# myungsub/meta-interpolation

Measured on AMD Instinct MI355X. Metric: inner-loop steps/sec, higher is better.
Workload: dtype f32 (3x3 convolutions: Winograd F(4x4) / F(2x2) on exact-f32 MFMAs, csrc/winograd4.h + winograd.hip; weight gradients and 5x5 / 7x7 / direct layers on csrc/convk*.hip: bf16x6 split operands, f32 accumulate; 51-tap op on 8-bit frames: exact integer frames x bf16x3 split taps, f32 accumulate); 1 GPU; c2_sepconv_256x448_b4_s5; plugin=sepconv, tasks_per_gpu=4, global_meta_batch=4, inner_steps=5, frame=256x448x3, inner_rule=lslr+SGD, seeded_weights=default, parallelism=task-parallel x1, 1 all-reduce of outer grads

## Files before the change

### meta-interpolation_amd/csrc/convk_wgrad.hip

```cpp
#include "common.h"
#include <stdlib.h>
#include <algorithm>

typedef float f32x4 __attribute__((ext_vector_type(4)));
typedef short bf16x8 __attribute__((ext_vector_type(8)));
typedef short bf16x4 __attribute__((ext_vector_type(4)));
typedef unsigned u32x4 __attribute__((ext_vector_type(4)));
typedef int i32x4 __attribute__((ext_vector_type(4)));
__device__ float ckw_raw_buffer_load_f32(i32x4 rsrc, int voffset, int soffset, int aux) __asm("llvm.amdgcn.raw.buffer.load.f32");

namespace {

constexpr int WG_THREADS = 256;
constexpr int UR = 4, UW = 32;

__device__ __forceinline__ i32x4 ckw_rsrc(const void* base, unsigned bytes) {
  const unsigned long long p = reinterpret_cast<unsigned long long>(base);
  i32x4 r;
  r.x = (int)(unsigned)p;
  r.y = (int)(unsigned)(p >> 32);
  r.z = (int)bytes;
  r.w = 0x00020000;
  return r;
}
// ... 570 lines not shown
  else wgrad_reduce_block(partial, gw, n, splits, blockIdx.x);
}

struct WgPlan { int mt, nt, ng, cobs, cibs, units, upr, ups, splits, ups_per_split, form; };

inline int savfi_cu_count() {
  static int cus[32] = {0};
  int dev = 0;
  if (hipGetDevice(&dev) != hipSuccess) return 256;
  int& n = cus[dev & 31];
  if (n == 0) {
    int v = 0;
    n = (hipDeviceGetAttribute(&v, hipDeviceAttributeMultiprocessorCount, dev) == hipSuccess && v > 0) ? v : 256;
  }
  return n;
}

inline int wg_plan(WgPlan& p, int N, int T, int Ci, int Co, int H, int W, int K, int pad, bool precise) {
  if (N <= 0 || T <= 0 || Ci <= 0 || Co <= 0 || H <= 0 || W <= 0 || N % T != 0 || pad < 0 || pad > K - 1) return SAVFI_E_SHAPE;
  if (K != 3 && K != 5 && K != 7) return SAVFI_E_UNSUPPORTED;
  const int Ho = H + 2 * pad - K + 1, Wo = W + 2 * pad - K + 1;
  if (Ho <= 0 || Wo <= 0) return SAVFI_E_SHAPE;
  if ((int64_t)Ci * H * W >= (1ll << 29) || (int64_t)Co * Ho * Wo >= (1ll << 29)) return SAVFI_E_TOOBIG;
  p.mt = (K == 3 && Co >= 192) ? 4 : 2;
#ifdef SAVFI_WGRAD_MT4
  if (K == 3 && Co >= SAVFI_WGRAD_MT4) p.mt = 4;
#endif
  p.nt = 1;
#if defined(SAVFI_WGRAD_NT) && SAVFI_WGRAD_NT == 2
  if (!precise && K != 7 && p.mt == 2 && Ci > 16) p.nt = 2;
#endif
  p.ng = 1;
#if defined(SAVFI_WGRAD_NG) && SAVFI_WGRAD_NG == 2
  if (K == 3 && p.mt == 4 && !precise && Ci >= 32) p.ng = 2;
#endif
#ifndef SAVFI_WGRAD3_FORM
#define SAVFI_WGRAD3_FORM 2
#endif
  p.form = (K == 3 && !precise && Co >= 48 && Ci >= 48 && SAVFI_WGRAD3_FORM == 2) ? 2 : 0;
  if (p.form) { p.mt = 4; p.nt = 4; p.ng = 1; }
  p.cobs = (Co + 16 * p.mt - 1) / (16 * p.mt);
  p.cibs = (Ci + 16 * p.nt * p.ng - 1) / (16 * p.nt * p.ng);
  const int ur = p.form == 2 ? ring::UR2 : UR;
  p.upr = (Ho + ur - 1) / ur;
  p.ups = (Wo + UW - 1) / UW;
  p.units = (N / T) * p.upr * p.ups;
  const int blocks = T * p.cobs * p.cibs;
  int splits;
#ifndef SAVFI_WGRAD_TARGET
#define SAVFI_WGRAD_TARGET 0
#endif
  constexpr int target = SAVFI_WGRAD_TARGET;
  if (target > 0) {
    splits = (target + blocks - 1) / blocks;
  } else {
    const int per_cu = (p.ng == 2 || p.form) ? 1 : (K == 3 && p.mt == 2 && p.nt == 1 && !precise) ? 3 : 2;
    const int64_t slots = (int64_t)per_cu * savfi_cu_count();
    double best_cost = 0.0;
    splits = 1;
    const int smax = (int)std::min<int64_t>(p.units, 4 * slots / blocks + 1);
    for (int sp = 1; sp <= smax; ++sp) {
      const int ups = (p.units + sp - 1) / sp;
      if ((p.units + ups - 1) / ups != sp) continue;
      const int64_t rounds = ((int64_t)blocks * sp + slots - 1) / slots;
      const double cost = p.form == 2 ? (double)rounds * (ups + 3.0) + 0.12 * sp : (double)rounds * (ups + 1.0) + 0.06 * sp;
      if (sp == 1 || cost < best_cost) { best_cost = cost; splits = sp; }
    }
  }
  if (splits > p.units) splits = p.units;
  if (splits < 1) splits = 1;
  p.ups_per_split = (p.units + splits - 1) / splits;
  p.splits = (p.units + p.ups_per_split - 1) / p.ups_per_split;
  return SAVFI_OK;
}

int launch_wgrad3_ring(const WgArgs& a, int blocks, float* bias_partial, hipStream_t stream) {
  static uint32_t configured = 0, configured_b = 0;
  const int rc = bias_partial ? savfi_ensure_dynamic_lds(reinterpret_cast<const void*>(convk_wgrad3_ring<true>), ring::LDS, configured_b)
                              : savfi_ensure_dynamic_lds(reinterpret_cast<const void*>(convk_wgrad3_ring<false>), ring::LDS, configured);
  if (rc != SAVFI_OK) return rc;
  if (bias_partial) hipLaunchKernelGGL(convk_wgrad3_ring<true>, dim3(blocks), dim3(ring::NTHR), ring::LDS, stream, a, bias_partial);
  else hipLaunchKernelGGL(convk_wgrad3_ring<false>, dim3(blocks), dim3(ring::NTHR), ring::LDS, stream, a, bias_partial);
  return savfi_launch_status();
}

template <int KS, int MT, int NT, bool P2 = false, int NG = 1>
int launch_wgrad(const WgArgs& a, int blocks, hipStream_t stream) {
  using G = WgGeom<KS, MT, NT * NG>;
  static uint32_t configured = 0;
  auto kern = convk_wgrad_kernel<KS, MT, NT, P2, NG>;
  if (G::LDS > 64 * 1024) {
    const int rc = savfi_ensure_dynamic_lds(reinterpret_cast<const void*>(kern), G::LDS, configured);
    if (rc != SAVFI_OK) return rc;
  }
  hipLaunchKernelGGL(kern, dim3(blocks), dim3(WG_THREADS * NG), G::LDS, stream, a);
  return savfi_launch_status();
}

}

extern "C" int64_t savfi_convk_wgrad_workspace_floats(int N, int T, int Ci, int Co, int H, int W, int K, int pad) {
  WgPlan p, q;
  int rc = wg_plan(p, N, T, Ci, Co, H, W, K, pad, false);
  if (rc != SAVFI_OK) return rc;
  rc = wg_plan(q, N, T, Ci, Co, H, W, K, pad, true);
  if (rc != SAVFI_OK) return rc;
  return (int64_t)(p.splits > q.splits ? p.splits : q.splits) * T * Co * (Ci * K * K + 1);
}

extern "C" int savfi_convk_wgrad_sums_bias(int N, int T, int Ci, int Co, int H, int W, int K, int pad) {
  WgPlan p;
  return wg_plan(p, N, T, Ci, Co, H, W, K, pad, false) == SAVFI_OK && p.form == 2 ? 1 : 0;
}

extern "C" int savfi_convk_wgrad_tasks_f32(const float* x, const float* gz, float* gw, float* workspace, int N, int T, int Ci, int Co,
                                           int H, int W, int K, int pad, int precise, void* stream) {
  return savfi_convk_wgrad_tasks_reflect_f32(x, gz, gw, workspace, N, T, Ci, Co, H, W, K, pad, precise, 0, stream);
}

namespace {
int convk_wgrad_run(const float* x, const float* gz, float* gw, float* gb, float* workspace, int N, int T, int Ci, int Co, int H, int W, int K,
                    int pad, int precise, int reflect, void* stream);
}

extern "C" int savfi_convk_wgrad_tasks_reflect_f32(const float* x, const float* gz, float* gw, float* workspace, int N, int T, int Ci,
                                                   int Co, int H, int W, int K, int pad, int precise, int reflect, void* stream) {
  return convk_wgrad_run(x, gz, gw, nullptr, workspace, N, T, Ci, Co, H, W, K, pad, precise, reflect, stream);
}

extern "C" int savfi_convk_wgrad_tasks_bias_f32(const float* x, const float* gz, float* gw, float* gb, float* workspace, int N, int T, int Ci,
                                                int Co, int H, int W, int K, int pad, int reflect, void* stream) {
  if (!gb) return SAVFI_E_NULL;
  if (!savfi_convk_wgrad_sums_bias(N, T, Ci, Co, H, W, K, pad)) return SAVFI_E_UNSUPPORTED;
  return convk_wgrad_run(x, gz, gw, gb, workspace, N, T, Ci, Co, H, W, K, pad, 0, reflect, stream);
}

namespace {
int convk_wgrad_run(const float* x, const float* gz, float* gw, float* gb, float* workspace, int N, int T, int Ci, int Co, int H, int W, int K,
                    int pad, int precise, int reflect, void* stream) {
  if (reflect && (pad >= H || pad >= W)) return SAVFI_E_UNSUPPORTED;
  if (!x || !gz || !gw || !workspace) return SAVFI_E_NULL;
  WgPlan p;
  int rc = wg_plan(p, N, T, Ci, Co, H, W, K, pad, precise != 0);
  if (rc != SAVFI_OK) return rc;
  WgArgs a;
  a.x = x; a.gz = gz; a.partial = workspace;
  a.N = N; a.T = T; a.Ci = Ci; a.Co = Co; a.H = H; a.W = W; a.pad = pad; a.reflect = reflect ? 1 : 0;
  a.Ho = H + 2 * pad - K + 1; a.Wo = W + 2 * pad - K + 1;
  a.cobs = p.cobs; a.cibs = p.cibs; a.splits = p.splits; a.units = p.units; a.units_per_split = p.ups_per_split;
  a.upr = p.upr; a.ups = p.ups;
  const int blocks = T * p.cobs * p.cibs * p.splits;
  hipStream_t st = (hipStream_t)stream;
  float* bias_partial = gb ? workspace + (size_t)p.splits * T * Co * Ci * K * K : nullptr;
  if (p.form == 2) rc = launch_wgrad3_ring(a, blocks, bias_partial, st);
  else if (K == 3 && precise) rc = p.mt == 4 ? launch_wgrad<3, 4, 1, true>(a, blocks, st) : launch_wgrad<3, 2, 1, true>(a, blocks, st);
  else if (K == 3 && p.ng == 2) rc = launch_wgrad<3, 4, 1, false, 2>(a, blocks, st);
  else if (K == 3) rc = p.mt == 4 ? launch_wgrad<3, 4, 1>(a, blocks, st) : p.nt == 2 ? launch_wgrad<3, 2, 2>(a, blocks, st) : launch_wgrad<3, 2, 1>(a, blocks, st);
  else if (K == 5) rc = precise ? launch_wgrad<5, 2, 1, true>(a, blocks, st) : p.nt == 2 ? launch_wgrad<5, 2, 2>(a, blocks, st) : launch_wgrad<5, 2, 1>(a, blocks, st);
  else rc = launch_wgrad<7, 2, 1>(a, blocks, st);
  if (rc != SAVFI_OK) return rc;
  const long long n = (long long)T * Co * Ci * K * K;
  const bool v4 = n % 4 == 0 && (((uintptr_t)workspace | (uintptr_t)gw) & 15u) == 0;
  const long long nb = gb ? (long long)T * Co : 0;
  const unsigned main_blocks = (unsigned)(v4 ? (n / 4 + 31) / 32 : (n + 31) / 32), bias_blocks = (unsigned)((nb + 31) / 32);
  if (v4) hipLaunchKernelGGL(convk_wgrad_reduce<true>, dim3(main_blocks + bias_blocks), dim3(256), 0, st, workspace, gw, n, p.splits, main_blocks, bias_partial, gb, nb);
  else hipLaunchKernelGGL(convk_wgrad_reduce<false>, dim3(main_blocks + bias_blocks), dim3(256), 0, st, workspace, gw, n, p.splits, main_blocks, bias_partial, gb, nb);
  return savfi_launch_status();
}
}
```

### meta-interpolation_amd/csrc/wgrad.hip

```cpp
#include "common.h"

namespace {

typedef float f32x4 __attribute__((ext_vector_type(4)));

constexpr int GNT = 256;
constexpr int GCO = 32, GCI = 32, GSEG = 64;
constexpr int GP = 68;
constexpr int G_FLOATS = GCO * GP;
constexpr int X_FLOATS = 3 * GCI * GP;
constexpr int BUF_FLOATS = G_FLOATS + X_FLOATS;
constexpr int TILE_FLOATS = 2 * 2 * 9 * 256;
constexpr int LDS_FLOATS_G = (2 * BUF_FLOATS > TILE_FLOATS) ? 2 * BUF_FLOATS : TILE_FLOATS;

struct WgradArgs {
  const float* x;
  const float* gz;
  float* partial;
  int Ci, Co, H, W, Ho, Wo, pad, rows, nseg, nrowchunk, cibs;
  int T;
};

struct Staged {
  float g[8], x[3][8], halo;
// ... 116 lines not shown
          acc[1][0][t] = __builtin_amdgcn_mfma_f32_16x16x4f32(ga1[ks], xs[0][ks + b], acc[1][0][t], 0, 0, 0);
          acc[1][1][t] = __builtin_amdgcn_mfma_f32_16x16x4f32(ga1[ks], xs[1][ks + b], acc[1][1][t], 0, 0, 0);
        }
    }
    store_rows(nxt, st, cols, tid, w);
    __syncthreads();
  }

  float* red = lds + lane * 4;
  for (int turn = 0; turn < 4; ++turn) {
    if (w == turn) {
#pragma unroll
      for (int rb = 0; rb < 2; ++rb)
#pragma unroll
        for (int cb = 0; cb < 2; ++cb)
#pragma unroll
          for (int t = 0; t < 9; ++t) {
            float* p = red + ((rb * 2 + cb) * 9 + t) * 256;
            f32x4 v = acc[rb][cb][t];
            if (turn > 0) v += *reinterpret_cast<const f32x4*>(p);
            if (turn < 3) *reinterpret_cast<f32x4*>(p) = v;
            else acc[rb][cb][t] = v;
          }
    }
    __syncthreads();
  }
  if (w == 3) {
    float* out = a.partial + (((size_t)blockIdx.z * gridDim.x + blockIdx.x) * gridDim.y + blockIdx.y) * TILE_FLOATS + lane * 4;
#pragma unroll
    for (int rb = 0; rb < 2; ++rb)
#pragma unroll
      for (int cb = 0; cb < 2; ++cb)
#pragma unroll
        for (int t = 0; t < 9; ++t) *reinterpret_cast<f32x4*>(out + ((rb * 2 + cb) * 9 + t) * 256) = acc[rb][cb][t];
  }
}

constexpr int RG = 16;
__global__ __launch_bounds__(256) void wgrad_reduce1(const float* __restrict__ partial, float* __restrict__ stage2,
                                                     size_t block_floats, int nsplit) {
  const size_t e4 = (size_t)blockIdx.x * 256 + threadIdx.x;
  if (e4 * 4 >= block_floats) return;
  partial += (size_t)blockIdx.z * nsplit * block_floats;
  stage2 += (size_t)blockIdx.z * gridDim.y * block_floats;
  const int s0 = blockIdx.y * RG, s1 = min(s0 + RG, nsplit);
  f32x4 acc = {0.f, 0.f, 0.f, 0.f};
  for (int sp = s0; sp < s1; ++sp) acc += *reinterpret_cast<const f32x4*>(partial + (size_t)sp * block_floats + e4 * 4);
  *reinterpret_cast<f32x4*>(stage2 + (size_t)blockIdx.y * block_floats + e4 * 4) = acc;
}

__global__ __launch_bounds__(256) void wgrad_reduce2(const float* __restrict__ stage2, float* __restrict__ gw, int Co, int Ci,
                                                     int cibs, int ntiles, int ngroups) {
  const int e = blockIdx.x * 256 + threadIdx.x;
  if (e >= Co * Ci * 9) return;
  stage2 += (size_t)blockIdx.y * ngroups * ntiles * TILE_FLOATS;
  gw += (size_t)blockIdx.y * Co * Ci * 9;
  const int tap = e % 9, ci = (e / 9) % Ci, co = e / (9 * Ci);
  const int cob = co >> 5, cib = ci >> 5, rb = (co >> 4) & 1, cb = (ci >> 4) & 1;
  const int row = co & 15, col = ci & 15, lane = (row >> 2) * 16 + col, reg = row & 3;
  const size_t off = (size_t)(cob * cibs + cib) * TILE_FLOATS + ((rb * 2 + cb) * 9 + tap) * 256 + lane * 4 + reg;
  float s = 0.f;
  for (int g = 0; g < ngroups; ++g) s += stage2[(size_t)g * ntiles * TILE_FLOATS + off];
  gw[e] = s;
}

struct WgradPlan {
  int Ho, Wo, cobs, cibs, nseg, rows, nrowchunk, ngroups;
  int64_t splits, partial_floats, stage2_floats;
};

bool wgrad_plan(WgradPlan& p, int N, int T, int Ci, int Co, int H, int W, int pad) {
  p.Ho = H + 2 * pad - 2;
  p.Wo = W + 2 * pad - 2;
  if (p.Ho <= 0 || p.Wo <= 0) return false;
  p.cobs = savfi_cdiv(Co, GCO);
  p.cibs = savfi_cdiv(Ci, GCI);
  p.nseg = savfi_cdiv(p.Wo, GSEG);
  const int64_t per_row = (int64_t)N * p.nseg * p.cobs * p.cibs;
  int best_rows = p.Ho;
  double best_cost = -1.0;
  for (int chunks = 1; chunks <= 128; ++chunks) {
    const int rows = savfi_cdiv(p.Ho, chunks);
    if (rows < 4 && chunks > 1) break;
    const int64_t wgs = per_row * savfi_cdiv(p.Ho, rows);
    const double cost = (double)((wgs + 511) / 512) * (rows + 3) + 0.004 * (double)wgs;
    if (best_cost < 0 || cost < best_cost) { best_cost = cost; best_rows = rows; }
  }
  p.rows = best_rows;
  p.nrowchunk = savfi_cdiv(p.Ho, best_rows);
  p.splits = (int64_t)(N / T) * p.nrowchunk * p.nseg;
  p.partial_floats = (int64_t)T * p.splits * p.cobs * p.cibs * TILE_FLOATS;
  p.ngroups = (int)((p.splits + RG - 1) / RG);
  p.stage2_floats = (int64_t)T * p.ngroups * p.cobs * p.cibs * TILE_FLOATS;
  return true;
}

}

extern "C" int64_t savfi_conv3x3_wgrad_tasks_workspace_floats(int N, int T, int Ci, int Co, int H, int W, int pad) {
  if (N <= 0 || T <= 0 || N % T != 0 || Ci <= 0 || Co <= 0 || H <= 0 || W <= 0) return SAVFI_E_SHAPE;
  if (pad != 0 && pad != 1) return SAVFI_E_UNSUPPORTED;
  WgradPlan p;
  if (!wgrad_plan(p, N, T, Ci, Co, H, W, pad)) return SAVFI_E_SHAPE;
  return p.partial_floats + p.stage2_floats;
}

extern "C" int64_t savfi_conv3x3_wgrad_workspace_floats(int N, int Ci, int Co, int H, int W, int pad) {
  return savfi_conv3x3_wgrad_tasks_workspace_floats(N, 1, Ci, Co, H, W, pad);
}

extern "C" int savfi_conv3x3_wgrad_tasks_f32(const float* x, const float* gz, float* gw, float* workspace, int N, int T, int Ci,
                                             int Co, int H, int W, int pad, void* stream) {
  if (!x || !gz || !gw || !workspace) return SAVFI_E_NULL;
  if (N <= 0 || T <= 0 || N % T != 0 || Ci <= 0 || Co <= 0 || H <= 0 || W <= 0) return SAVFI_E_SHAPE;
  if (pad != 0 && pad != 1) return SAVFI_E_UNSUPPORTED;
  WgradPlan p;
  if (!wgrad_plan(p, N, T, Ci, Co, H, W, pad)) return SAVFI_E_SHAPE;
  if ((int64_t)Ci * H * W >= ((int64_t)1 << 29) || (int64_t)Co * p.Ho * p.Wo >= ((int64_t)1 << 29)) return SAVFI_E_TOOBIG;
  if (p.ngroups > 65535 || p.splits > 0x7fffffffLL || (int64_t)p.cobs * p.cibs > 65535 || (int64_t)Co * Ci * 9 > 0x7fffffffLL || T > 65535) return SAVFI_E_TOOBIG;
  hipStream_t st = (hipStream_t)stream;
  constexpr size_t lds = (size_t)LDS_FLOATS_G * sizeof(float);
  static uint32_t attr_done = 0;
  if (int e = savfi_ensure_dynamic_lds((const void*)wgrad3x3, lds, attr_done)) return e;
  WgradArgs a{x, gz, workspace, Ci, Co, H, W, p.Ho, p.Wo, pad, p.rows, p.nseg, p.nrowchunk, p.cibs, T};
  hipLaunchKernelGGL(wgrad3x3, dim3((unsigned)p.splits, p.cobs * p.cibs, T), dim3(GNT), lds, st, a);
  if (int e = savfi_launch_status()) return e;
  const int ntiles = p.cobs * p.cibs;
  const size_t block_floats = (size_t)ntiles * TILE_FLOATS;
  float* stage2 = workspace + p.partial_floats;
  if (p.ngroups == 1) {
    hipLaunchKernelGGL(wgrad_reduce2, dim3(savfi_cdiv(Co * Ci * 9, 256), T), dim3(256), 0, st, workspace, gw, Co, Ci, p.cibs, ntiles,
                       (int)p.splits);
    return savfi_launch_status();
  }
  hipLaunchKernelGGL(wgrad_reduce1, dim3((unsigned)((block_floats / 4 + 255) / 256), p.ngroups, T), dim3(256), 0, st, workspace,
                     stage2, block_floats, (int)p.splits);
  if (int e = savfi_launch_status()) return e;
  hipLaunchKernelGGL(wgrad_reduce2, dim3(savfi_cdiv(Co * Ci * 9, 256), T), dim3(256), 0, st, stage2, gw, Co, Ci, p.cibs, ntiles,
                     p.ngroups);
  return savfi_launch_status();
}

extern "C" int savfi_conv3x3_wgrad_f32(const float* x, const float* gz, float* gw, float* workspace, int N, int Ci, int Co,
                                       int H, int W, int pad, void* stream) {
  return savfi_conv3x3_wgrad_tasks_f32(x, gz, gw, workspace, N, 1, Ci, Co, H, W, pad, stream);
}

namespace {

typedef int i32x4w __attribute__((ext_vector_type(4)));
typedef float f32x2w __attribute__((ext_vector_type(2)));

constexpr int WW_TK = 8;
constexpr int WW_PY = WW_TK * 4 + 4;
constexpr int WW_CB = 32;
constexpr int WW_HALF = 4 * WW_CB * WW_PY;
constexpr int WW_BUF = 2 * WW_HALF;
constexpr int WW_BLOCK_FLOATS = WW_CB * WW_CB * 9;
#ifndef WW_DOUBLE
#define WW_DOUBLE 0
#endif
constexpr int WW_LDS_FLOATS = (WW_DOUBLE ? 2 : 1) * WW_BUF;

struct WWArgs {
  const float* x;
  const float* gz;
  float* partial;
  int Ci, Co, H, W, Ho, Wo, pad, T, cibs;
  int ty_cnt, tx_cnt, cpr;
  int chunks_total;
  int chunks_per_split;
  float* bias_partial;
};

}

__device__ f32x4 savfi_wg_buffer_load_x4(i32x4w rsrc, int voffset, int soffset, int aux) __asm("llvm.amdgcn.raw.buffer.load.v4f32");
__device__ f32x2w savfi_wg_buffer_load_x2(i32x4w rsrc, int voffset, int soffset, int aux) __asm("llvm.amdgcn.raw.buffer.load.v2f32");

namespace {

__device__ __forceinline__ i32x4w ww_rsrc(const float* base, unsigned bytes) {
  const unsigned long long p = reinterpret_cast<unsigned long long>(base);
  i32x4w r;
  r.x = (int)(unsigned)p; r.y = (int)(unsigned)(p >> 32); r.z = (int)bytes; r.w = 0x00020000;
  return r;
}

struct WWChunk {
  float d[16];
  float g[4];
  int cx;
};

constexpr unsigned WW_OOR = 0x40000000u;
struct WWPos {
  int nq, ty, cx;
  unsigned xrow[4], grow[2];
};

__device__ __forceinline__ void ww_set_row(WWPos& p, const WWArgs& a) {
#pragma unroll
  for (int r = 0; r < 4; ++r) {
    const int y = 2 * p.ty - a.pad + r;
    p.xrow[r] = (y >= 0 && y < a.H) ? (unsigned)(y * a.W) * 4u : WW_OOR;
  }
#pragma unroll
  for (int u = 0; u < 2; ++u) {
    const int y = 2 * p.ty + u;
    p.grow[u] = y < a.Ho ? (unsigned)(y * a.Wo) * 4u : WW_OOR;
  }
}

__device__ __forceinline__ void ww_load(WWChunk& c, const WWArgs& a, const WWPos& p, int task, int tl, unsigned xplane, unsigned gplane) {
  const int n = p.nq * a.T + task;
  const int tx = p.cx * WW_TK + tl;
  const i32x4w xr = ww_rsrc(a.x + (size_t)n * a.Ci * a.H * a.W, (unsigned)(a.Ci * a.H * a.W) * 4u);
  const int x0 = 2 * tx - a.pad;
  c.cx = p.cx;
  const unsigned xoff = xplane + (unsigned)max(x0, 0) * 4u;
#pragma unroll
  for (int r = 0; r < 4; ++r) {
    const f32x4 v = savfi_wg_buffer_load_x4(xr, (int)xoff, (int)p.xrow[r], 0);
    c.d[4 * r] = v.x; c.d[4 * r + 1] = v.y; c.d[4 * r + 2] = v.z; c.d[4 * r + 3] = v.w;
  }
  const i32x4w gr = ww_rsrc(a.gz + (size_t)n * a.Co * a.Ho * a.Wo, (unsigned)(a.Co * a.Ho * a.Wo) * 4u);
  const unsigned goff = 2 * tx < a.Wo ? gplane + (unsigned)(2 * tx) * 4u : WW_OOR;
#pragma unroll
  for (int u = 0; u < 2; ++u) {
    const f32x2w v = savfi_wg_buffer_load_x2(gr, (int)goff, (int)p.grow[u], 0);
    c.g[2 * u] = v.x; c.g[2 * u + 1] = v.y;
  }
}

__device__ __forceinline__ void ww_transform_store(WWChunk& c, const WWArgs& a, float* __restrict__ ybuf, float* __restrict__ vbuf, int ch, int tl,
                                                   float* __restrict__ bias_acc) {
  float (&d)[16] = c.d;
  if (c.cx == 0 && a.pad > 0) {
    if (tl == 0) {
#pragma unroll
      for (int r = 0; r < 4; ++r) { d[4 * r + 3] = d[4 * r + 2]; d[4 * r + 2] = d[4 * r + 1]; d[4 * r + 1] = d[4 * r]; d[4 * r] = 0.f; }
    }
  }
  if (c.cx == a.cpr - 1) {
    const int tx = c.cx * WW_TK + tl;
    const int wcols = a.W - (2 * tx - a.pad), gcols = a.Wo - 2 * tx;
#pragma unroll
    for (int r = 0; r < 4; ++r) {
      d[4 * r] = wcols > 0 ? d[4 * r] : 0.f;
      d[4 * r + 1] = wcols > 1 ? d[4 * r + 1] : 0.f;
      d[4 * r + 2] = wcols > 2 ? d[4 * r + 2] : 0.f;
      d[4 * r + 3] = wcols > 3 ? d[4 * r + 3] : 0.f;
    }
    c.g[1] = gcols > 1 ? c.g[1] : 0.f;
    c.g[3] = gcols > 1 ? c.g[3] : 0.f;
  }
  float t[16];
#pragma unroll
  for (int cc = 0; cc < 4; ++cc) {
    t[cc] = d[cc] - d[8 + cc];
    t[4 + cc] = d[4 + cc] + d[8 + cc];
    t[8 + cc] = d[8 + cc] - d[4 + cc];
    t[12 + cc] = d[4 + cc] - d[12 + cc];
  }
#pragma unroll
  for (int r = 0; r < 4; ++r)
    *reinterpret_cast<f32x4*>(vbuf + (r * WW_CB + ch) * WW_PY + 4 * tl) =
        (f32x4){t[4 * r] - t[4 * r + 2], t[4 * r + 1] + t[4 * r + 2], t[4 * r + 2] - t[4 * r + 1], t[4 * r + 1] - t[4 * r + 3]};
  const float g00 = c.g[0], g01 = c.g[1], g10 = c.g[2], g11 = c.g[3];
  if (bias_acc) *bias_acc += (g00 + g01) + (g10 + g11);
  const float s0[2] = {g00, g01}, s1[2] = {g00 + g10, g01 + g11}, s2[2] = {g00 - g10, g01 - g11}, s3[2] = {g10, g11};
  *reinterpret_cast<f32x4*>(ybuf + (0 * WW_CB + ch) * WW_PY + 4 * tl) = (f32x4){s0[0], s0[0] + s0[1], s0[0] - s0[1], s0[1]};
  *reinterpret_cast<f32x4*>(ybuf + (1 * WW_CB + ch) * WW_PY + 4 * tl) = (f32x4){s1[0], s1[0] + s1[1], s1[0] - s1[1], s1[1]};
  *reinterpret_cast<f32x4*>(ybuf + (2 * WW_CB + ch) * WW_PY + 4 * tl) = (f32x4){s2[0], s2[0] + s2[1], s2[0] - s2[1], s2[1]};
  *reinterpret_cast<f32x4*>(ybuf + (3 * WW_CB + ch) * WW_PY + 4 * tl) = (f32x4){s3[0], s3[0] + s3[1], s3[0] - s3[1], s3[1]};
}

template <bool BIAS>
__global__ __launch_bounds__(256, WW_DOUBLE ? 2 : 4) void wino_wgrad3x3(WWArgs a) {
  extern __shared__ __attribute__((aligned(16))) float lds[];
  const int tid = threadIdx.x, lane = tid & 63, w = __builtin_amdgcn_readfirstlane(tid >> 6);
  const int tl = tid & 7, ch = tid >> 3;
  const int task = blockIdx.z;
  const int cob = blockIdx.y / a.cibs, cib = blockIdx.y - cob * a.cibs;
  const int q0 = blockIdx.x * a.chunks_per_split, q1 = min(q0 + a.chunks_per_split, a.chunks_total);
  const int ci = cib * WW_CB + ch, co = cob * WW_CB + ch;

  f32x4 acc[4][2][2];
#pragma unroll
  for (int c = 0; c < 4; ++c)
#pragma unroll
    for (int i = 0; i < 2; ++i)
#pragma unroll
      for (int j = 0; j < 2; ++j) acc[c][i][j] = (f32x4){0.f, 0.f, 0.f, 0.f};

  const int frag = (w * WW_CB + (lane & 15)) * WW_PY + 4 * (lane >> 4);
  WWChunk cur;
  WWPos pos;
  {
    const int per_img = a.ty_cnt * a.cpr;
    pos.nq = q0 / per_img;
    const int rem = q0 - pos.nq * per_img;
    pos.ty = rem / a.cpr;
    pos.cx = rem - pos.ty * a.cpr;
  }
  const unsigned xplane = ci < a.Ci ? (unsigned)(ci * a.H * a.W) * 4u : WW_OOR;
  const unsigned gplane = co < a.Co ? (unsigned)(co * a.Ho * a.Wo) * 4u : WW_OOR;
  ww_set_row(pos, a);
  if (q0 < q1) ww_load(cur, a, pos, task, tl, xplane, gplane);
  const bool do_bias = BIAS && cib == 0;
  auto bias_slot = [&]() { return lds + WW_LDS_FLOATS + threadIdx.x; };
  if (do_bias) *bias_slot() = 0.f;
  for (int q = q0; q < q1; ++q) {
    float* buf = lds + (WW_DOUBLE ? ((q - q0) & 1) * WW_BUF : 0);
    if (!WW_DOUBLE && q != q0) __syncthreads();
    ww_transform_store(cur, a, buf, buf + WW_HALF, ch, tl, do_bias ? bias_slot() : nullptr);
    if (q + 1 < q1) {
      if (++pos.cx == a.cpr) {
        pos.cx = 0;
        if (++pos.ty == a.ty_cnt) { pos.ty = 0; ++pos.nq; }
        ww_set_row(pos, a);
      }
      ww_load(cur, a, pos, task, tl, xplane, gplane);
    }
    __builtin_amdgcn_sched_barrier(0);
    __syncthreads();
    const float* yb = buf + frag;
    const float* vb = buf + WW_HALF + frag;
#pragma unroll
    for (int ks = 0; ks < WW_TK / 4; ++ks) {
      f32x4 ya[2], va[2];
#pragma unroll
      for (int i = 0; i < 2; ++i) {
        ya[i] = *reinterpret_cast<const f32x4*>(yb + 16 * i * WW_PY + 16 * ks);
        va[i] = *reinterpret_cast<const f32x4*>(vb + 16 * i * WW_PY + 16 * ks);
      }
#pragma unroll
      for (int c = 0; c < 4; ++c)
#pragma unroll
        for (int i = 0; i < 2; ++i)
#pragma unroll
          for (int j = 0; j < 2; ++j) acc[c][i][j] = __builtin_amdgcn_mfma_f32_16x16x4f32(ya[i][c], va[j][c], acc[c][i][j], 0, 0, 0);
      __builtin_amdgcn_sched_barrier(0);
    }
  }
  __syncthreads();
  if (do_bias) {
    auto dpp = [](float v, auto ctrl) {
      return __builtin_bit_cast(float, __builtin_amdgcn_update_dpp(0, __builtin_bit_cast(int, v), decltype(ctrl)::value, 0xf, 0xf, true));
    };
    float bsum = *bias_slot();
    bsum += dpp(bsum, std::integral_constant<int, 0xB1>{});
    bsum += dpp(bsum, std::integral_constant<int, 0x4E>{});
    bsum += dpp(bsum, std::integral_constant<int, 0x141>{});
    if (tl == 0) a.bias_partial[(((size_t)task * gridDim.x + blockIdx.x) * (gridDim.y / a.cibs) + cob) * WW_CB + ch] = bsum;
  }

  const float sr = (w == 1 || w == 2) ? 0.5f : 1.f;
  float* ex = lds;
  float* out = a.partial + (((size_t)task * gridDim.x + blockIdx.x) * gridDim.y + blockIdx.y) * WW_BLOCK_FLOATS;
#pragma unroll
  for (int i = 0; i < 2; ++i) {
#pragma unroll
    for (int j = 0; j < 2; ++j) {
      f32x4 u0, u1, u2;
#pragma unroll
      for (int e = 0; e < 4; ++e) {
        const float m0 = acc[0][i][j][e], m1 = acc[1][i][j][e], m2 = acc[2][i][j][e], m3 = acc[3][i][j][e];
        const float h = 0.5f * (m1 + m2);
        u0[e] = sr * (m0 + h);
        u1[e] = sr * (0.5f * (m1 - m2));
        u2[e] = sr * (h - m3);
      }
      float* p = ex + ((w * 3) * 2 + j) * 256 + lane * 4;
      *reinterpret_cast<f32x4*>(p) = u0;
      *reinterpret_cast<f32x4*>(p + 2 * 256) = u1;
      *reinterpret_cast<f32x4*>(p + 4 * 256) = u2;
    }
    __syncthreads();
    for (int item = tid; item < 3 * 2 * 256; item += 256) {
      const int reg = item & 3, ln = (item >> 2) & 63, j = (item >> 8) & 1, b = item >> 9;
      const float* p = ex + (b * 2 + j) * 256 + ln * 4 + reg;
      const float u_0 = p[0], u_1 = p[3 * 2 * 256], u_2 = p[2 * 3 * 2 * 256], u_3 = p[3 * 3 * 2 * 256];
      const int cor = 16 * i + 4 * (ln >> 4) + reg, cic = 16 * j + (ln & 15);
      float* o = out + (cor * WW_CB + cic) * 9 + b;
      o[0] = u_0 + u_1 + u_2;
      o[3] = u_1 - u_2;
      o[6] = u_1 + u_2 - u_3;
    }
    __syncthreads();
  }
}

__global__ __launch_bounds__(256) void wino_wgrad_reduce2(const float* __restrict__ stage2, float* __restrict__ gw, int Co, int Ci,
                                                          int cibs, int ntiles, int ngroups) {
  const int e = blockIdx.x * 256 + threadIdx.x;
  if (e >= Co * Ci * 9) return;
  stage2 += (size_t)blockIdx.y * ngroups * ntiles * WW_BLOCK_FLOATS;
  gw += (size_t)blockIdx.y * Co * Ci * 9;
  const int k = e % 9, ci = (e / 9) % Ci, co = e / (9 * Ci);
  const size_t off = (size_t)((co / WW_CB) * cibs + ci / WW_CB) * WW_BLOCK_FLOATS + ((co % WW_CB) * WW_CB + ci % WW_CB) * 9 + k;
  float s = 0.f;
  for (int g = 0; g < ngroups; ++g) s += stage2[(size_t)g * ntiles * WW_BLOCK_FLOATS + off];
  gw[e] = s;
}

__global__ __launch_bounds__(64) void wino_wgrad_bias_reduce(const float* __restrict__ bias_partial, float* __restrict__ gb, int Co, int cobs,
                                                             int nsplit) {
  const int co = blockIdx.x * 64 + threadIdx.x, task = blockIdx.y;
  if (co >= Co) return;
  const float* p = bias_partial + (size_t)task * nsplit * cobs * WW_CB + co;
  float s = 0.f;
  for (int sp = 0; sp < nsplit; ++sp) s += p[(size_t)sp * cobs * WW_CB];
  gb[(size_t)task * Co + co] = s;
}

struct WWPlan {
  int Ho, Wo, cobs, cibs, ty_cnt, tx_cnt, cpr, chunks_total, chunks_per_split, nsplit, ngroups;
  int64_t partial_floats, stage2_floats;
};

bool ww_plan(WWPlan& p, int N, int T, int Ci, int Co, int H, int W, int pad) {
  p.Ho = H + 2 * pad - 2;
  p.Wo = W + 2 * pad - 2;
  if (p.Ho <= 0 || p.Wo <= 0) return false;
  p.cobs = savfi_cdiv(Co, WW_CB);
  p.cibs = savfi_cdiv(Ci, WW_CB);
  p.ty_cnt = savfi_cdiv(p.Ho, 2);
  p.tx_cnt = savfi_cdiv(p.Wo, 2);
  p.cpr = savfi_cdiv(p.tx_cnt, WW_TK);
  const int64_t chunks = (int64_t)(N / T) * p.ty_cnt * p.cpr;
  if (chunks > 0x7fffffffLL) return false;
  p.chunks_total = (int)chunks;
  const int64_t blocks = (int64_t)T * p.cobs * p.cibs;
  int64_t want = (512 * 2 + blocks - 1) / blocks;
#ifndef SAVFI_WWGRAD_MIN_CHUNKS
#define SAVFI_WWGRAD_MIN_CHUNKS 16
#endif
  constexpr int min_chunks = SAVFI_WWGRAD_MIN_CHUNKS;
  const int64_t most = chunks / min_chunks > 0 ? chunks / min_chunks : 1;
  if (want > most) want = most;
  if (want < 1) want = 1;
  p.chunks_per_split = savfi_cdiv(chunks, want);
  p.nsplit = savfi_cdiv(chunks, p.chunks_per_split);
  p.ngroups = savfi_cdiv(p.nsplit, RG);
  p.partial_floats = (int64_t)T * p.nsplit * p.cobs * p.cibs * WW_BLOCK_FLOATS;
  p.stage2_floats = (int64_t)T * p.ngroups * p.cobs * p.cibs * WW_BLOCK_FLOATS;
  return true;
}

}

extern "C" int64_t savfi_conv3x3_wgrad_wino_tasks_workspace_floats(int N, int T, int Ci, int Co, int H, int W, int pad) {
  if (N <= 0 || T <= 0 || N % T != 0 || Ci <= 0 || Co <= 0 || H <= 0 || W <= 0) return SAVFI_E_SHAPE;
  if (pad != 0 && pad != 1) return SAVFI_E_UNSUPPORTED;
  WWPlan p;
  if (!ww_plan(p, N, T, Ci, Co, H, W, pad)) return SAVFI_E_SHAPE;
  return p.partial_floats + p.stage2_floats;
}

extern "C" int64_t savfi_conv3x3_wgrad_wino_tasks_bias_workspace_floats(int N, int T, int Ci, int Co, int H, int W, int pad) {
  const int64_t base = savfi_conv3x3_wgrad_wino_tasks_workspace_floats(N, T, Ci, Co, H, W, pad);
  if (base < 0) return base;
  WWPlan p;
  ww_plan(p, N, T, Ci, Co, H, W, pad);
  return base + (int64_t)T * p.nsplit * p.cobs * WW_CB;
}

static int wino_wgrad_tasks(const float* x, const float* gz, float* gw, float* gb, float* workspace, int N, int T, int Ci, int Co, int H,
                            int W, int pad, void* stream);

extern "C" int savfi_conv3x3_wgrad_wino_tasks_f32(const float* x, const float* gz, float* gw, float* workspace, int N, int T,
                                                  int Ci, int Co, int H, int W, int pad, void* stream) {
  return wino_wgrad_tasks(x, gz, gw, nullptr, workspace, N, T, Ci, Co, H, W, pad, stream);
}

extern "C" int savfi_conv3x3_wgrad_wino_tasks_bias_f32(const float* x, const float* gz, float* gw, float* gb, float* workspace, int N, int T,
                                                       int Ci, int Co, int H, int W, int pad, void* stream) {
  if (!gb) return SAVFI_E_NULL;
  return wino_wgrad_tasks(x, gz, gw, gb, workspace, N, T, Ci, Co, H, W, pad, stream);
}

static int wino_wgrad_tasks(const float* x, const float* gz, float* gw, float* gb, float* workspace, int N, int T, int Ci, int Co, int H,
                            int W, int pad, void* stream) {
  if (!x || !gz || !gw || !workspace) return SAVFI_E_NULL;
  if (N <= 0 || T <= 0 || N % T != 0 || Ci <= 0 || Co <= 0 || H <= 0 || W <= 0) return SAVFI_E_SHAPE;
  if (pad != 0 && pad != 1) return SAVFI_E_UNSUPPORTED;
  WWPlan p;
  if (!ww_plan(p, N, T, Ci, Co, H, W, pad)) return SAVFI_E_SHAPE;
  if ((int64_t)Ci * H * W >= ((int64_t)1 << 28) || (int64_t)Co * p.Ho * p.Wo >= ((int64_t)1 << 28)) return SAVFI_E_TOOBIG;
  if (p.ngroups > 65535 || (int64_t)p.cobs * p.cibs > 65535 || (int64_t)Co * Ci * 9 > 0x7fffffffLL || T > 65535) return SAVFI_E_TOOBIG;
  hipStream_t st = (hipStream_t)stream;
  constexpr size_t lds = (size_t)WW_LDS_FLOATS * sizeof(float), lds_bias = lds + 256 * sizeof(float);
  static uint32_t attr_done = 0, attr_done_b = 0;
  if (int e = gb ? savfi_ensure_dynamic_lds((const void*)wino_wgrad3x3<true>, lds_bias, attr_done_b)
                 : savfi_ensure_dynamic_lds((const void*)wino_wgrad3x3<false>, lds, attr_done)) return e;
  float* bias_partial = gb ? workspace + p.partial_floats + p.stage2_floats : nullptr;
  WWArgs a{x, gz, workspace, Ci, Co, H, W, p.Ho, p.Wo, pad, T, p.cibs, p.ty_cnt, p.tx_cnt, p.cpr, p.chunks_total, p.chunks_per_split,
           bias_partial};
  if (gb) hipLaunchKernelGGL(wino_wgrad3x3<true>, dim3(p.nsplit, p.cobs * p.cibs, T), dim3(256), lds_bias, st, a);
  else hipLaunchKernelGGL(wino_wgrad3x3<false>, dim3(p.nsplit, p.cobs * p.cibs, T), dim3(256), lds, st, a);
  if (int e = savfi_launch_status()) return e;
  if (gb) {
    hipLaunchKernelGGL(wino_wgrad_bias_reduce, dim3(savfi_cdiv(Co, 64), T), dim3(64), 0, st, bias_partial, gb, Co, p.cobs, p.nsplit);
    if (int e = savfi_launch_status()) return e;
  }
  const int ntiles = p.cobs * p.cibs;
  const size_t block_floats = (size_t)ntiles * WW_BLOCK_FLOATS;
  float* stage2 = workspace + p.partial_floats;
  if (p.ngroups == 1) {
    hipLaunchKernelGGL(wino_wgrad_reduce2, dim3(savfi_cdiv(Co * Ci * 9, 256), T), dim3(256), 0, st, workspace, gw, Co, Ci, p.cibs, ntiles,
                       p.nsplit);
    return savfi_launch_status();
  }
  hipLaunchKernelGGL(wgrad_reduce1, dim3((unsigned)((block_floats / 4 + 255) / 256), p.ngroups, T), dim3(256), 0, st, workspace,
                     stage2, block_floats, p.nsplit);
  if (int e = savfi_launch_status()) return e;
  hipLaunchKernelGGL(wino_wgrad_reduce2, dim3(savfi_cdiv(Co * Ci * 9, 256), T), dim3(256), 0, st, stage2, gw, Co, Ci, p.cibs, ntiles,
                     p.ngroups);
  return savfi_launch_status();
}
```

Before: 248.1 inner-loop steps/sec.

## Write wgrad directly when unsplit, swizzle LDS tiles, fuse bias and main reductions

When the plan uses a single split, both the Winograd and the convk weight-gradient kernels now write gradients and bias straight into gw/gb, so the workspace partials and the reduce launch are skipped. The Winograd LDS row padding is replaced by an XOR swizzle of the tile index, which keeps bank conflicts low while shrinking LDS. The separate bias-reduce kernel is folded into the main reduction kernel as extra blocks. Splits up to a threshold are now reduced in one pass with grouped summation instead of going through the two-stage path. The costs are new bounds checks on the direct store path and different summation orders.

```diff
diff --git a/meta-interpolation_amd/csrc/convk_wgrad.hip b/meta-interpolation_amd/csrc/convk_wgrad.hip
--- a/meta-interpolation_amd/csrc/convk_wgrad.hip
+++ b/meta-interpolation_amd/csrc/convk_wgrad.hip
@@ -746,13 +746,15 @@
   const int blocks = T * p.cobs * p.cibs * p.splits;
   hipStream_t st = (hipStream_t)stream;
   float* bias_partial = gb ? workspace + (size_t)p.splits * T * Co * Ci * K * K : nullptr;
+  const bool direct = p.splits == 1;
+  if (direct) { a.partial = gw; if (gb) bias_partial = gb; }
   if (p.form == 2) rc = launch_wgrad3_ring(a, blocks, bias_partial, st);
   else if (K == 3 && precise) rc = p.mt == 4 ? launch_wgrad<3, 4, 1, true>(a, blocks, st) : launch_wgrad<3, 2, 1, true>(a, blocks, st);
   else if (K == 3 && p.ng == 2) rc = launch_wgrad<3, 4, 1, false, 2>(a, blocks, st);
   else if (K == 3) rc = p.mt == 4 ? launch_wgrad<3, 4, 1>(a, blocks, st) : p.nt == 2 ? launch_wgrad<3, 2, 2>(a, blocks, st) : launch_wgrad<3, 2, 1>(a, blocks, st);
   else if (K == 5) rc = precise ? launch_wgrad<5, 2, 1, true>(a, blocks, st) : p.nt == 2 ? launch_wgrad<5, 2, 2>(a, blocks, st) : launch_wgrad<5, 2, 1>(a, blocks, st);
   else rc = launch_wgrad<7, 2, 1>(a, blocks, st);
-  if (rc != SAVFI_OK) return rc;
+  if (rc != SAVFI_OK || direct) return rc;
   const long long n = (long long)T * Co * Ci * K * K;
   const bool v4 = n % 4 == 0 && (((uintptr_t)workspace | (uintptr_t)gw) & 15u) == 0;
   const long long nb = gb ? (long long)T * Co : 0;
diff --git a/meta-interpolation_amd/csrc/wgrad.hip b/meta-interpolation_amd/csrc/wgrad.hip
--- a/meta-interpolation_amd/csrc/wgrad.hip
+++ b/meta-interpolation_amd/csrc/wgrad.hip
@@ -292,7 +292,8 @@
 typedef float f32x2w __attribute__((ext_vector_type(2)));
 
 constexpr int WW_TK = 8;
-constexpr int WW_PY = WW_TK * 4 + 4;
+constexpr int WW_PY = WW_TK * 4;
+static_assert(WW_TK == 8, "the tile swizzle (channel >> 1) & 7 covers eight tiles");
 constexpr int WW_CB = 32;
 constexpr int WW_HALF = 4 * WW_CB * WW_PY;
 constexpr int WW_BUF = 2 * WW_HALF;
@@ -306,6 +307,8 @@
   const float* x;
   const float* gz;
   float* partial;
+  float* gw_direct;
+  float* gb_direct;
   int Ci, Co, H, W, Ho, Wo, pad, T, cibs;
   int ty_cnt, tx_cnt, cpr;
   int chunks_total;
@@ -374,7 +377,7 @@
 }
 
 __device__ __forceinline__ void ww_transform_store(WWChunk& c, const WWArgs& a, float* __restrict__ ybuf, float* __restrict__ vbuf, int ch, int tl,
-                                                   float* __restrict__ bias_acc) {
+                                                   int tls, float* __restrict__ bias_acc) {
   float (&d)[16] = c.d;
   if (c.cx == 0 && a.pad > 0) {
     if (tl == 0) {
@@ -405,15 +408,15 @@
   }
 #pragma unroll
   for (int r = 0; r < 4; ++r)
-    *reinterpret_cast<f32x4*>(vbuf + (r * WW_CB + ch) * WW_PY + 4 * tl) =
+    *reinterpret_cast<f32x4*>(vbuf + (r * WW_CB + ch) * WW_PY + tls) =
         (f32x4){t[4 * r] - t[4 * r + 2], t[4 * r + 1] + t[4 * r + 2], t[4 * r + 2] - t[4 * r + 1], t[4 * r + 1] - t[4 * r + 3]};
   const float g00 = c.g[0], g01 = c.g[1], g10 = c.g[2], g11 = c.g[3];
   if (bias_acc) *bias_acc += (g00 + g01) + (g10 + g11);
   const float s0[2] = {g00, g01}, s1[2] = {g00 + g10, g01 + g11}, s2[2] = {g00 - g10, g01 - g11}, s3[2] = {g10, g11};
-  *reinterpret_cast<f32x4*>(ybuf + (0 * WW_CB + ch) * WW_PY + 4 * tl) = (f32x4){s0[0], s0[0] + s0[1], s0[0] - s0[1], s0[1]};
-  *reinterpret_cast<f32x4*>(ybuf + (1 * WW_CB + ch) * WW_PY + 4 * tl) = (f32x4){s1[0], s1[0] + s1[1], s1[0] - s1[1], s1[1]};
-  *reinterpret_cast<f32x4*>(ybuf + (2 * WW_CB + ch) * WW_PY + 4 * tl) = (f32x4){s2[0], s2[0] + s2[1], s2[0] - s2[1], s2[1]};
-  *reinterpret_cast<f32x4*>(ybuf + (3 * WW_CB + ch) * WW_PY + 4 * tl) = (f32x4){s3[0], s3[0] + s3[1], s3[0] - s3[1], s3[1]};
+  *reinterpret_cast<f32x4*>(ybuf + (0 * WW_CB + ch) * WW_PY + tls) = (f32x4){s0[0], s0[0] + s0[1], s0[0] - s0[1], s0[1]};
+  *reinterpret_cast<f32x4*>(ybuf + (1 * WW_CB + ch) * WW_PY + tls) = (f32x4){s1[0], s1[0] + s1[1], s1[0] - s1[1], s1[1]};
+  *reinterpret_cast<f32x4*>(ybuf + (2 * WW_CB + ch) * WW_PY + tls) = (f32x4){s2[0], s2[0] + s2[1], s2[0] - s2[1], s2[1]};
+  *reinterpret_cast<f32x4*>(ybuf + (3 * WW_CB + ch) * WW_PY + tls) = (f32x4){s3[0], s3[0] + s3[1], s3[0] - s3[1], s3[1]};
 }
 
 template <bool BIAS>
@@ -421,6 +424,7 @@
   extern __shared__ __attribute__((aligned(16))) float lds[];
   const int tid = threadIdx.x, lane = tid & 63, w = __builtin_amdgcn_readfirstlane(tid >> 6);
   const int tl = tid & 7, ch = tid >> 3;
+  const int tls = 4 * (tl ^ ((ch >> 1) & 7));
   const int task = blockIdx.z;
   const int cob = blockIdx.y / a.cibs, cib = blockIdx.y - cob * a.cibs;
   const int q0 = blockIdx.x * a.chunks_per_split, q1 = min(q0 + a.chunks_per_split, a.chunks_total);
@@ -434,7 +438,7 @@
 #pragma unroll
       for (int j = 0; j < 2; ++j) acc[c][i][j] = (f32x4){0.f, 0.f, 0.f, 0.f};
 
-  const int frag = (w * WW_CB + (lane & 15)) * WW_PY + 4 * (lane >> 4);
+  const int frag = (w * WW_CB + (lane & 15)) * WW_PY + 4 * ((lane >> 4) ^ (((lane & 15) >> 1) & 7));
   WWChunk cur;
   WWPos pos;
   {
@@ -454,7 +458,7 @@
   for (int q = q0; q < q1; ++q) {
     float* buf = lds + (WW_DOUBLE ? ((q - q0) & 1) * WW_BUF : 0);
     if (!WW_DOUBLE && q != q0) __syncthreads();
-    ww_transform_store(cur, a, buf, buf + WW_HALF, ch, tl, do_bias ? bias_slot() : nullptr);
+    ww_transform_store(cur, a, buf, buf + WW_HALF, ch, tl, tls, do_bias ? bias_slot() : nullptr);
     if (q + 1 < q1) {
       if (++pos.cx == a.cpr) {
         pos.cx = 0;
@@ -465,15 +469,15 @@
     }
     __builtin_amdgcn_sched_barrier(0);
     __syncthreads();
-    const float* yb = buf + frag;
-    const float* vb = buf + WW_HALF + frag;
 #pragma unroll
     for (int ks = 0; ks < WW_TK / 4; ++ks) {
+      const float* yb = buf + (frag ^ (16 * ks));
+      const float* vb = yb + WW_HALF;
       f32x4 ya[2], va[2];
 #pragma unroll
       for (int i = 0; i < 2; ++i) {
-        ya[i] = *reinterpret_cast<const f32x4*>(yb + 16 * i * WW_PY + 16 * ks);
-        va[i] = *reinterpret_cast<const f32x4*>(vb + 16 * i * WW_PY + 16 * ks);
+        ya[i] = *reinterpret_cast<const f32x4*>(yb + 16 * i * WW_PY);
+        va[i] = *reinterpret_cast<const f32x4*>(vb + 16 * i * WW_PY);
       }
 #pragma unroll
       for (int c = 0; c < 4; ++c)
@@ -493,12 +497,20 @@
     bsum += dpp(bsum, std::integral_constant<int, 0xB1>{});
     bsum += dpp(bsum, std::integral_constant<int, 0x4E>{});
     bsum += dpp(bsum, std::integral_constant<int, 0x141>{});
-    if (tl == 0) a.bias_partial[(((size_t)task * gridDim.x + blockIdx.x) * (gridDim.y / a.cibs) + cob) * WW_CB + ch] = bsum;
+    if (a.gb_direct) {
+      if (tl == 0 && co < a.Co) a.gb_direct[(size_t)task * a.Co + co] = bsum;
+    } else if (tl == 0) {
+      a.bias_partial[(((size_t)task * gridDim.x + blockIdx.x) * (gridDim.y / a.cibs) + cob) * WW_CB + ch] = bsum;
+    }
   }
 
   const float sr = (w == 1 || w == 2) ? 0.5f : 1.f;
   float* ex = lds;
-  float* out = a.partial + (((size_t)task * gridDim.x + blockIdx.x) * gridDim.y + blockIdx.y) * WW_BLOCK_FLOATS;
+  const bool direct = a.gw_direct != nullptr;
+  float* out = direct ? a.gw_direct + ((size_t)task * a.Co + cob * WW_CB) * a.Ci * 9 + (size_t)cib * WW_CB * 9
+                      : a.partial + (((size_t)task * gridDim.x + blockIdx.x) * gridDim.y + blockIdx.y) * WW_BLOCK_FLOATS;
+  const int opitch = direct ? a.Ci * 9 : WW_CB * 9;
+  const int co_left = direct ? a.Co - cob * WW_CB : WW_CB, ci_left = direct ? a.Ci - cib * WW_CB : WW_CB;
 #pragma unroll
   for (int i = 0; i < 2; ++i) {
 #pragma unroll
@@ -523,36 +535,46 @@
       const float* p = ex + (b * 2 + j) * 256 + ln * 4 + reg;
       const float u_0 = p[0], u_1 = p[3 * 2 * 256], u_2 = p[2 * 3 * 2 * 256], u_3 = p[3 * 3 * 2 * 256];
       const int cor = 16 * i + 4 * (ln >> 4) + reg, cic = 16 * j + (ln & 15);
-      float* o = out + (cor * WW_CB + cic) * 9 + b;
-      o[0] = u_0 + u_1 + u_2;
-      o[3] = u_1 - u_2;
-      o[6] = u_1 + u_2 - u_3;
+      if (cor < co_left && cic < ci_left) {
+        float* o = out + (size_t)cor * opitch + cic * 9 + b;
+        o[0] = u_0 + u_1 + u_2;
+        o[3] = u_1 - u_2;
+        o[6] = u_1 + u_2 - u_3;
+      }
     }
     __syncthreads();
   }
 }
 
-__global__ __launch_bounds__(256) void wino_wgrad_reduce2(const float* __restrict__ stage2, float* __restrict__ gw, int Co, int Ci,
-                                                          int cibs, int ntiles, int ngroups) {
+constexpr int WW_ONE_PASS_MAX = 4 * RG;
+__global__ __launch_bounds__(256) void wino_wgrad_reduce(const float* __restrict__ blocks, float* __restrict__ gw, int Co, int Ci, int cibs,
+                                                         int ntiles, int nblocks, int group, unsigned main_blocks,
+                                                         const float* __restrict__ bias_partial, float* __restrict__ gb, int cobs, int nsplit) {
+  const int task = blockIdx.y;
+  if (blockIdx.x >= main_blocks) {
+    const int co = (blockIdx.x - main_blocks) * 256 + threadIdx.x;
+    if (co >= Co) return;
+    const float* p = bias_partial + (size_t)task * nsplit * cobs * WW_CB + co;
+    float s = 0.f;
+    for (int sp = 0; sp < nsplit; ++sp) s += p[(size_t)sp * cobs * WW_CB];
+    gb[(size_t)task * Co + co] = s;
+    return;
+  }
   const int e = blockIdx.x * 256 + threadIdx.x;
   if (e >= Co * Ci * 9) return;
-  stage2 += (size_t)blockIdx.y * ngroups * ntiles * WW_BLOCK_FLOATS;
-  gw += (size_t)blockIdx.y * Co * Ci * 9;
+  blocks += (size_t)task * nblocks * ntiles * WW_BLOCK_FLOATS;
+  gw += (size_t)task * Co * Ci * 9;
   const int k = e % 9, ci = (e / 9) % Ci, co = e / (9 * Ci);
   const size_t off = (size_t)((co / WW_CB) * cibs + ci / WW_CB) * WW_BLOCK_FLOATS + ((co % WW_CB) * WW_CB + ci % WW_CB) * 9 + k;
+  const size_t stride = (size_t)ntiles * WW_BLOCK_FLOATS;
   float s = 0.f;
-  for (int g = 0; g < ngroups; ++g) s += stage2[(size_t)g * ntiles * WW_BLOCK_FLOATS + off];
+  for (int g0 = 0; g0 < nblocks; g0 += group) {
+    const int g1 = min(g0 + group, nblocks);
+    float inner = 0.f;
+    for (int sp = g0; sp < g1; ++sp) inner += blocks[(size_t)sp * stride + off];
+    s += inner;
+  }
   gw[e] = s;
-}
-
-__global__ __launch_bounds__(64) void wino_wgrad_bias_reduce(const float* __restrict__ bias_partial, float* __restrict__ gb, int Co, int cobs,
-                                                             int nsplit) {
-  const int co = blockIdx.x * 64 + threadIdx.x, task = blockIdx.y;
-  if (co >= Co) return;
-  const float* p = bias_partial + (size_t)task * nsplit * cobs * WW_CB + co;
-  float s = 0.f;
-  for (int sp = 0; sp < nsplit; ++sp) s += p[(size_t)sp * cobs * WW_CB];
-  gb[(size_t)task * Co + co] = s;
 }
 
 struct WWPlan {
@@ -636,27 +658,26 @@
   if (int e = gb ? savfi_ensure_dynamic_lds((const void*)wino_wgrad3x3<true>, lds_bias, attr_done_b)
                  : savfi_ensure_dynamic_lds((const void*)wino_wgrad3x3<false>, lds, attr_done)) return e;
   float* bias_partial = gb ? workspace + p.partial_floats + p.stage2_floats : nullptr;
-  WWArgs a{x, gz, workspace, Ci, Co, H, W, p.Ho, p.Wo, pad, T, p.cibs, p.ty_cnt, p.tx_cnt, p.cpr, p.chunks_total, p.chunks_per_split,
-           bias_partial};
+  const bool direct = p.nsplit == 1;
+  WWArgs a{x, gz, workspace, direct ? gw : nullptr, direct ? gb : nullptr, Ci, Co, H, W, p.Ho, p.Wo, pad, T, p.cibs, p.ty_cnt, p.tx_cnt, p.cpr,
+           p.chunks_total, p.chunks_per_split, bias_partial};
   if (gb) hipLaunchKernelGGL(wino_wgrad3x3<true>, dim3(p.nsplit, p.cobs * p.cibs, T), dim3(256), lds_bias, st, a);
   else hipLaunchKernelGGL(wino_wgrad3x3<false>, dim3(p.nsplit, p.cobs * p.cibs, T), dim3(256), lds, st, a);
   if (int e = savfi_launch_status()) return e;
-  if (gb) {
-    hipLaunchKernelGGL(wino_wgrad_bias_reduce, dim3(savfi_cdiv(Co, 64), T), dim3(64), 0, st, bias_partial, gb, Co, p.cobs, p.nsplit);
-    if (int e = savfi_launch_status()) return e;
-  }
+  if (direct) return SAVFI_OK;
   const int ntiles = p.cobs * p.cibs;
   const size_t block_floats = (size_t)ntiles * WW_BLOCK_FLOATS;
   float* stage2 = workspace + p.partial_floats;
-  if (p.ngroups == 1) {
-    hipLaunchKernelGGL(wino_wgrad_reduce2, dim3(savfi_cdiv(Co * Ci * 9, 256), T), dim3(256), 0, st, workspace, gw, Co, Ci, p.cibs, ntiles,
-                       p.nsplit);
+  const unsigned main_blocks = (unsigned)savfi_cdiv(Co * Ci * 9, 256), bias_blocks = gb ? (unsigned)savfi_cdiv(Co, 256) : 0u;
+  if (p.nsplit <= WW_ONE_PASS_MAX) {
+    hipLaunchKernelGGL(wino_wgrad_reduce, dim3(main_blocks + bias_blocks, T), dim3(256), 0, st, workspace, gw, Co, Ci, p.cibs, ntiles, p.nsplit,
+                       RG, main_blocks, bias_partial, gb, p.cobs, p.nsplit);
     return savfi_launch_status();
   }
   hipLaunchKernelGGL(wgrad_reduce1, dim3((unsigned)((block_floats / 4 + 255) / 256), p.ngroups, T), dim3(256), 0, st, workspace,
                      stage2, block_floats, p.nsplit);
   if (int e = savfi_launch_status()) return e;
-  hipLaunchKernelGGL(wino_wgrad_reduce2, dim3(savfi_cdiv(Co * Ci * 9, 256), T), dim3(256), 0, st, stage2, gw, Co, Ci, p.cibs, ntiles,
-                     p.ngroups);
+  hipLaunchKernelGGL(wino_wgrad_reduce, dim3(main_blocks + bias_blocks, T), dim3(256), 0, st, stage2, gw, Co, Ci, p.cibs, ntiles, p.ngroups,
+                     p.ngroups, main_blocks, bias_partial, gb, p.cobs, p.nsplit);
   return savfi_launch_status();
 }
```

Result: no change. 251.0 inner-loop steps/sec, median of 3 (+1.2%).
